# abdur75648/AI-Camera

Measured on AMD Instinct MI355X. Metric: end-to-end frames/sec @1280x720, 30 persons/frame, higher is better.
Workload: dtype f16

## Files before the change

### ai-camera_amd/csrc/conv_common.hpp

```cpp
#pragma once
#include "kernels.hpp"

#include <cstdlib>
#include <type_traits>
#include <utility>

namespace aic {

typedef _Float16 half8 __attribute__((ext_vector_type(8)));
typedef _Float16 half4 __attribute__((ext_vector_type(4)));
typedef float floatx4 __attribute__((ext_vector_type(4)));

__device__ __forceinline__ float act_apply(float v, int act) {
    if (act == 1) return v / (1.0f + __expf(-v));
    if (act == 2) return fmaxf(v, 0.0f);
    return v;
}

template <typename T> struct Frag;
template <> struct Frag<half_t> {
    typedef half8 type;
    static __device__ __forceinline__ floatx4 mma(const half8& a, const half8& b, floatx4 c) {
        return __builtin_amdgcn_mfma_f32_16x16x32_f16(a, b, c, 0, 0, 0);
    }
};
template <> struct Frag<float> {
    typedef floatx4 type;
    static __device__ __forceinline__ floatx4 partial(const floatx4& a, const floatx4& b) {
        floatx4 p = {0.f, 0.f, 0.f, 0.f};
        p = __builtin_amdgcn_mfma_f32_16x16x4f32(a[0], b[0], p, 0, 0, 0);
        p = __builtin_amdgcn_mfma_f32_16x16x4f32(a[1], b[1], p, 0, 0, 0);
        p = __builtin_amdgcn_mfma_f32_16x16x4f32(a[2], b[2], p, 0, 0, 0);
        p = __builtin_amdgcn_mfma_f32_16x16x4f32(a[3], b[3], p, 0, 0, 0);
        return p;
    }
    static __device__ __forceinline__ floatx4 mma(const floatx4& a, const floatx4& b, floatx4 c) { return c + partial(a, b); }
};

template <typename T, int MT, int NT>
__device__ __forceinline__ void mma_tiles(floatx4 (&acc)[MT][NT], const typename Frag<T>::type (&wf)[NT], const typename Frag<T>::type (&xf)[MT]) {
    if constexpr (sizeof(T) == 2) {
#pragma unroll
        for (int i = 0; i < MT; ++i)
#pragma unroll
            for (int j = 0; j < NT; ++j) acc[i][j] = Frag<T>::mma(wf[j], xf[i], acc[i][j]);
    } else {
        floatx4 prev = Frag<T>::partial(wf[0], xf[0]);
        __builtin_amdgcn_sched_barrier(0);
#pragma unroll
        for (int t = 1; t < MT * NT; ++t) {
            const floatx4 p = Frag<T>::partial(wf[t % NT], xf[t / NT]);
            acc[(t - 1) / NT][(t - 1) % NT] += prev;
            asm volatile("" : "+v"(acc[(t - 1) / NT][(t - 1) % NT]));
            prev = p;
            __builtin_amdgcn_sched_barrier(0);
        }
        acc[MT - 1][NT - 1] += prev;
        asm volatile("" : "+v"(acc[MT - 1][NT - 1]));
    }
}

constexpr int MID_STEPS = 16;
template <int MT, int NT>
__device__ __forceinline__ void mma_tiles_mid(floatx4 (&mid)[MT][NT], const floatx4 (&wf)[NT], const floatx4 (&xf)[MT]) {
    floatx4 prev = Frag<float>::partial(wf[0], xf[0]);
    __builtin_amdgcn_sched_barrier(0);
#pragma unroll
    for (int t = 1; t < MT * NT; ++t) {
        const floatx4 p = Frag<float>::partial(wf[t % NT], xf[t / NT]);
        mid[(t - 1) / NT][(t - 1) % NT] += prev;
        asm volatile("" : "+v"(mid[(t - 1) / NT][(t - 1) % NT]));
        prev = p;
        __builtin_amdgcn_sched_barrier(0);
    }
    mid[MT - 1][NT - 1] += prev;
    asm volatile("" : "+v"(mid[MT - 1][NT - 1]));
}
typedef float doublex4 __attribute__((ext_vector_type(4)));
template <int MT, int NT>
__device__ __forceinline__ void flush_mid(doublex4 (&accd)[MT][NT], floatx4 (&mid)[MT][NT]) {
#pragma unroll
    for (int i = 0; i < MT; ++i)
#pragma unroll
        for (int j = 0; j < NT; ++j) {
#pragma unroll
            for (int e = 0; e < 4; ++e) accd[i][j][e] += mid[i][j][e];
            mid[i][j] = floatx4{0.f, 0.f, 0.f, 0.f};
        }
}

__device__ __forceinline__ int lds_swz(int row) { return ((row >> 1) & 3) ^ ((row >> 3) & 2); }
__device__ __forceinline__ int lds_off(int row, int chunk) { return row * 64 + 16 * (chunk ^ lds_swz(row)); }

__device__ __forceinline__ void fast_divmod(int m, int d, float inv, int& q, int& r) {
    q = (int)(__int2float_rz(m) * inv);
    r = m - q * d;
    if (r >= d) { r -= d; ++q; }
    if (r < 0) { r += d; --q; }
}

template <int ACT> __device__ __forceinline__ float act_fast(float v) {
    if constexpr (ACT == 1) {
        return v * __builtin_amdgcn_rcpf(1.0f + __builtin_amdgcn_exp2f(v * -1.4426950408889634f));
    } else if constexpr (ACT == 2) {
        return fmaxf(v, 0.0f);
    } else {
        return v;
    }
}

template <typename T, int ACT> __device__ __forceinline__ float act_t(float v) {
    if constexpr (sizeof(T) == 4 && ACT == 1) return v / (1.0f + expf(-v));
    else return act_fast<ACT>(v);
}

template <typename T, int MT, int NT, int ACT, int RES, bool F32OUT>
__device__ __forceinline__ void epilogue_fast(const ConvArgs& a, floatx4 (&acc)[MT][NT], const int (&mrow)[MT], int n_base, int q) {
    const float* __restrict__ bias = a.bias;
    const T* __restrict__ rg = reinterpret_cast<const T*>(a.res);
    floatx4 b4[NT];
    bool ncol[NT];
#pragma unroll
    for (int j = 0; j < NT; ++j) {
        const int n = n_base + j * 16 + 4 * q;
        ncol[j] = n < a.Cout;
        b4[j] = *reinterpret_cast<const floatx4*>(bias + n);
    }
#pragma unroll
    for (int i = 0; i < MT; ++i) {
        const int m = mrow[i];
        if (m < 0) continue;
        const size_t ybase = (size_t)m * a.y_cs + a.y_coff;
        const size_t rbase = RES ? (size_t)m * a.r_cs + a.r_coff : 0;
#pragma unroll
        for (int j = 0; j < NT; ++j) {
            if (!ncol[j]) continue;
            const int n = n_base + j * 16 + 4 * q;
            float v[4];
#pragma unroll
            for (int e = 0; e < 4; ++e) v[e] = acc[i][j][e] + b4[j][e];
            if constexpr (RES != 0) {
                float rv[4];
                if constexpr (sizeof(T) == 2) {
                    const half4 h = *reinterpret_cast<const half4*>(rg + rbase + n);
#pragma unroll
                    for (int e = 0; e < 4; ++e) rv[e] = (float)h[e];
                } else {
                    const floatx4 h = *reinterpret_cast<const floatx4*>(rg + rbase + n);
#pragma unroll
                    for (int e = 0; e < 4; ++e) rv[e] = h[e];
                }
#pragma unroll
                for (int e = 0; e < 4; ++e) v[e] = RES == 1 ? act_t<T, ACT>(v[e] + rv[e]) : act_t<T, ACT>(v[e]) + rv[e];
            } else {
// ... 292 lines not shown
#pragma unroll
            for (int e = 0; e < 4; ++e) own[e] = (half_t)act_fast<1>(acc[i][NT - 1][e] + b1[NT - 1][e]);
            const int2 u = *reinterpret_cast<const int2*>(&own);
            const int s0 = (((2 * q) & 3) * 16 + r) * 4, s1 = (((2 * q + 1) & 3) * 16 + r) * 4;
            int4 g;
            g.x = __builtin_amdgcn_ds_bpermute(s0, u.x), g.y = __builtin_amdgcn_ds_bpermute(s0, u.y);
            g.z = __builtin_amdgcn_ds_bpermute(s1, u.x), g.w = __builtin_amdgcn_ds_bpermute(s1, u.y);
            if (q >= 2) g = make_int4(0, 0, 0, 0);
            bf[NP] = *reinterpret_cast<const half8*>(&g);
        }
        floatx4 acc2[1][NT];
#pragma unroll
        for (int j = 0; j < NT; ++j) acc2[0][j] = floatx4{0.f, 0.f, 0.f, 0.f};
#pragma unroll
        for (int s = 0; s < KS; ++s)
#pragma unroll
            for (int j = 0; j < NT; ++j) acc2[0][j] = __builtin_amdgcn_mfma_f32_16x16x32_f16(wf[j][s], bf[s], acc2[0][j], 0, 0, 0);
        const int m1[1] = {mrow[i]};
        if (a.t_max) {
            floatx4 bt[NT];
#pragma unroll
            for (int p = 0; p < NP; ++p) {
                bt[2 * p] = *reinterpret_cast<const floatx4*>(a.b_tail + 32 * p + 8 * q);
                bt[2 * p + 1] = *reinterpret_cast<const floatx4*>(a.b_tail + 32 * p + 8 * q + 4);
            }
            if constexpr (NT & 1) bt[NT - 1] = *reinterpret_cast<const floatx4*>(a.b_tail + 16 * (NT - 1) + 4 * q);
            float best = -__builtin_inff();
            int arg = 0x7fffffff;
#pragma unroll
            for (int j = 0; j < NT; ++j)
#pragma unroll
                for (int e = 0; e < 4; ++e) {
                    const int ch = perm_ch<NT>(j, q, e);
                    const float v = acc2[0][j][e] + bt[j][e];
                    if (ch < a.t_cout && v > best) { best = v; arg = ch; }
                }
#pragma unroll
            for (int off = 16; off <= 32; off <<= 1) {
                const float ov = __shfl_xor(best, off);
                const int oa = __shfl_xor(arg, off);
                if (ov > best || (ov == best && oa < arg)) { best = ov; arg = oa; }
            }
            const int m = mrow[i];
            if (q == 0 && m >= 0) {
                const int im = m / a.t_hw;
                const size_t o = (size_t)im * a.t_na + a.t_a0 + (m - im * a.t_hw);
                a.t_max[o] = best;
                a.t_arg[o] = arg;
            }
        } else if (NT == 4 && a.t_box) {
            if constexpr (NT == 4) {
                floatx4 bt[4];
#pragma unroll
                for (int p = 0; p < 2; ++p) {
                    bt[2 * p] = *reinterpret_cast<const floatx4*>(a.b_tail + 32 * p + 8 * q);
                    bt[2 * p + 1] = *reinterpret_cast<const floatx4*>(a.b_tail + 32 * p + 8 * q + 4);
                }
                const bool odd = q & 1;
                float dist[2];
#pragma unroll
                for (int h = 0; h < 2; ++h) {
                    float v[8];
#pragma unroll
                    for (int k = 0; k < 8; ++k) v[k] = acc2[0][2 * h + (k >> 2)][k & 3] + bt[2 * h + (k >> 2)][k & 3];
                    float mx = v[0];
#pragma unroll
                    for (int k = 1; k < 8; ++k) mx = fmaxf(mx, v[k]);
                    mx = fmaxf(mx, __shfl_xor(mx, 16));
                    float e[8];
#pragma unroll
                    for (int k = 0; k < 8; ++k) e[k] = __builtin_amdgcn_exp2f((v[k] - mx) * 1.4426950408889634f);
                    float sum = 0.f, ex = 0.f;
                    if (!odd) {
#pragma unroll
                        for (int k = 0; k < 8; ++k) { sum += e[k]; ex += e[k] * (float)k; }
                    }
                    const float s_in = __shfl_xor(sum, 16), x_in = __shfl_xor(ex, 16);
                    if (odd) {
                        sum = s_in, ex = x_in;
#pragma unroll
                        for (int k = 0; k < 8; ++k) { sum += e[k]; ex += e[k] * (float)(8 + k); }
                    }
                    dist[h] = ex / sum;
                }
                const float d1 = __shfl_xor(dist[0], 32), d3 = __shfl_xor(dist[1], 32);
                const int m = mrow[i];
                if (q == 1 && m >= 0) {
                    const int im = m / a.t_hw, cell = m - im * a.t_hw;
                    const int gy = cell / a.t_w, gx = cell - gy * a.t_w;
                    const float cx = (float)gx + 0.5f, cy = (float)gy + 0.5f, st = (float)a.t_stride;
                    const size_t o = (size_t)im * a.t_na + a.t_a0 + cell;
                    *reinterpret_cast<floatx4*>(a.t_box + o * 4) = floatx4{(cx - dist[0]) * st, (cy - d1) * st, (cx + dist[1]) * st, (cy + d3) * st};
                }
            }
        } else {
            epilogue_dispatch<half_t, 1, NT, true>(a2, acc2, m1, 0, q);
        }
    }
}

typedef const __attribute__((address_space(1))) void* gptr_t;
typedef __attribute__((address_space(3))) void* lptr_t;


__device__ __forceinline__ int xcd_tile(int b, int nb, int on) {
    if (!on) return b;
    const int x = b & 7, base = nb >> 3, rem = nb & 7;
    return x * base + (x < rem ? x : rem) + (b >> 3);
}
__device__ __forceinline__ void xcd_tile_xy(int on, int& bx, int& by) {
    const int nbx = (int)gridDim.x, lin = (int)blockIdx.y * nbx + (int)blockIdx.x;
    const int t = xcd_tile(lin, nbx * (int)gridDim.y, on);
    by = t / nbx, bx = t - by * nbx;
}
__device__ __forceinline__ bool xcd_tile_xy_live(int on, int nbx_live, int& bx, int& by) {
    const int lin = (int)blockIdx.y * (int)gridDim.x + (int)blockIdx.x;
    const int nlive = nbx_live * (int)gridDim.y;
    if (lin >= nlive) return false;
    const int t = xcd_tile(lin, nlive, on);
    by = t / nbx_live, bx = t - by * nbx_live;
    return true;
}

template <int N> __device__ __forceinline__ void wait_vmcnt() {
    if constexpr (N == 0) asm volatile("s_waitcnt vmcnt(0)" ::: "memory");
    else if constexpr (N == 1) asm volatile("s_waitcnt vmcnt(1)" ::: "memory");
    else if constexpr (N == 2) asm volatile("s_waitcnt vmcnt(2)" ::: "memory");
    else if constexpr (N == 3) asm volatile("s_waitcnt vmcnt(3)" ::: "memory");
    else if constexpr (N == 4) asm volatile("s_waitcnt vmcnt(4)" ::: "memory");
    else if constexpr (N == 5) asm volatile("s_waitcnt vmcnt(5)" ::: "memory");
    else if constexpr (N == 6) asm volatile("s_waitcnt vmcnt(6)" ::: "memory");
    else if constexpr (N == 7) asm volatile("s_waitcnt vmcnt(7)" ::: "memory");
    else if constexpr (N == 8) asm volatile("s_waitcnt vmcnt(8)" ::: "memory");
    else if constexpr (N == 9) asm volatile("s_waitcnt vmcnt(9)" ::: "memory");
    else if constexpr (N == 10) asm volatile("s_waitcnt vmcnt(10)" ::: "memory");
    else if constexpr (N == 11) asm volatile("s_waitcnt vmcnt(11)" ::: "memory");
    else if constexpr (N == 12) asm volatile("s_waitcnt vmcnt(12)" ::: "memory");
    else if constexpr (N == 14) asm volatile("s_waitcnt vmcnt(14)" ::: "memory");
    else if constexpr (N == 15) asm volatile("s_waitcnt vmcnt(15)" ::: "memory");
    else if constexpr (N == 16) asm volatile("s_waitcnt vmcnt(16)" ::: "memory");
    else if constexpr (N == 18) asm volatile("s_waitcnt vmcnt(18)" ::: "memory");
    else if constexpr (N == 20) asm volatile("s_waitcnt vmcnt(20)" ::: "memory");
    else static_assert(N < 0, "add this vmcnt literal");
}


constexpr int ppp_ipix_pad(int th, int tw) {
    int ipix = (th + 2) * (tw + 2);
    if (tw >= 16) return ipix;
    while (ipix % 16 != tw && ipix % 16 != 16 - tw) ++ipix;
    return ipix;
}

__device__ __forceinline__ int lane_here() {
    int l;
    asm volatile("v_mbcnt_lo_u32_b32 %0, -1, 0\n\tv_mbcnt_hi_u32_b32 %0, -1, %0" : "=v"(l));
    return l;
}


void launch_conv_wide(const ConvArgs& a, const ConvPlan& p, hipStream_t s);
void launch_conv_pp(const ConvArgs& a, const ConvPlan& p, hipStream_t s);
void launch_conv_pp_patch(const ConvArgs& a, const ConvPlan& p, hipStream_t s);
void launch_conv_sp_patch(const ConvArgs& a, const ConvPlan& p, hipStream_t s);
void launch_conv_s2_patch(const ConvArgs& a, const ConvPlan& p, hipStream_t s);
void launch_conv_patch(const ConvArgs& a, const ConvPlan& p, hipStream_t s);
void launch_conv_pm_patch(const ConvArgs& a, const ConvPlan& p, hipStream_t s);
void launch_conv_c16(const ConvArgs& a, const ConvPlan& p, hipStream_t s);
void launch_conv_c32s2_tail(const ConvArgs& a, const ConvPlan& p, hipStream_t s);
void launch_conv_1x1_stream(const ConvArgs& a, const ConvPlan& p, hipStream_t s);
void launch_conv_c64_resident(const ConvArgs& a, const ConvPlan& p, hipStream_t s);

}
```

### ai-camera_amd/csrc/kernels_conv_sp.hip

```cpp
#include "conv_common.hpp"

namespace aic {

template <int MT, int NT, int WM, int WN, int TH, int TW>
__global__ __launch_bounds__(512) void conv3x3_sp_patch_kernel(const ConvArgs a, int ny, int run) {
    typedef half_t T;
    constexpr int NSTAGE = 4;
    constexpr int CH = 8, BKE = 32, RP = 128;
    constexpr int BM = WM * MT * 16;
    constexpr int BN = WN * NT * 16;
    constexpr int B_PER = BN / RP;
    constexpr int LPS = B_PER + 1;
    constexpr int TPIX = TH * TW, NI = BM / TPIX;
    constexpr int PW = TW + 2, PH = TH + 2, IPIX = PW * PH, IPIXP = ppp_ipix_pad(TH, TW), NPIX = NI * IPIXP;
    constexpr int G = TW >= 16 ? 1 : 16 / TW;
    constexpr int NPASS = (NPIX + 127) / 128, NPIXP = NPASS * 128;
    constexpr int PLANE = NPIXP * 16, PBUF = 4 * PLANE, WSTAGE = BN * 64;
    constexpr int PATCH0 = NSTAGE * WSTAGE, DUM0 = PATCH0 + 2 * PBUF;
    static_assert(WM * WN == 8 && MT == 8 && NT == 4 && BN % RP == 0 && BM % TPIX == 0 && NPASS <= 7 && TW % 4 == 0, "geometry");
    static_assert((NSTAGE - 1) * WSTAGE + 2048 < 65536 && PBUF + (2 * PW + 2 + IPIXP * NI) * 16 < 65536, "ds_read immediates");

    extern __shared__ __attribute__((aligned(16))) char smem[];

    const int t = threadIdx.x;
    const int lane = t & 63, wv = __builtin_amdgcn_readfirstlane(t >> 6);
    const int HW = a.H * a.W;
    const int n_img = a.n_dev ? min(a.M / HW, a.n_dev[0]) : a.M / HW;
    const int ntiles = ((n_img + NI - 1) / NI) * ny;
    const int nruns = (ntiles + run - 1) / run;
    if ((int)blockIdx.x >= nruns) return;
    int t_cur = xcd_tile((int)blockIdx.x, nruns, a.xcd_map) * run;
    const int t_end = min(t_cur + run, ntiles);
    int img0 = (t_cur / ny) * NI, n0 = (t_cur % ny) * BN;

    const T* __restrict__ xg = reinterpret_cast<const T*>(a.x);
    const T* __restrict__ wg = reinterpret_cast<const T*>(a.w);
    const T* zero = reinterpret_cast<const T*>(a.zero);

    const int plane = wv & 3;
    const T* pptr[NPASS];
    int pil[NPASS];
#pragma unroll
    for (int i = 0; i < NPASS; ++i) {
        const int p = i * 128 + (wv >> 2) * 64 + lane;
        const int il = p / IPIXP, rem = p - il * IPIXP;
        const int py = rem / PW, px = rem - py * PW;
        const int iy = py - 1, ix = px - 1;
        const bool ok = p < NPIX && rem < IPIX && (unsigned)iy < (unsigned)TH && (unsigned)ix < (unsigned)TW;
        pptr[i] = ok ? xg + ((size_t)((il * TH + iy) * TW + ix) * a.x_cs + a.x_coff + plane * CH) : zero;
        pil[i] = ok ? il : 0x40000000;
    }
    char* const pdst = smem + PATCH0 + plane * PLANE + (wv >> 2) * 1024;
    const unsigned img_bytes = (unsigned)HW * a.x_cs * 2u;
    const int slot = t & 3, r0 = t >> 2;
    const int kc = slot ^ lds_swz(r0);
    const T* wptr[B_PER];
#pragma unroll
    for (int j = 0; j < B_PER; ++j) wptr[j] = wg + (size_t)(r0 + RP * j) * a.Kp + kc * CH;
    char* const wdst = smem + (16 * wv) * 64;
    const int nchunks = a.Cin / BKE;
    const unsigned tile_wbytes = (unsigned)BN * a.Kp * 2u;
    const unsigned tap_bytes = (unsigned)a.Cin * 2u;

    unsigned long long w_off = (unsigned long long)(n0 / BN) * tile_wbytes;
    int w_c = 0;
    int n0_next = n0, img_next = img0;
    bool has_next = t_cur + 1 < t_end;
    if (has_next) { img_next = ((t_cur + 1) / ny) * NI; n0_next = ((t_cur + 1) % ny) * BN; }
    auto issue_w = [&](int st, int wtap) {
        char* sbase = wdst + st * WSTAGE;
#pragma unroll
        for (int j = 0; j < B_PER; ++j) {
            const T* src = reinterpret_cast<const T*>(reinterpret_cast<const char*>(wptr[j]) + w_off);
            asm volatile("" : "+v"(src));
            __builtin_amdgcn_global_load_lds((gptr_t)src, (lptr_t)(sbase + j * (RP * 64)), 16, 0, 0);
        }
        if (wtap < 8) w_off += tap_bytes;
        else {
            w_off += 64u - 8u * (unsigned long long)tap_bytes;
            if (++w_c == nchunks) {
                w_c = 0;
                w_off = (unsigned long long)((has_next ? n0_next : n0) / BN) * tile_wbytes;
            }
        }
    };
    unsigned long long p_off = 0;
    int p_lim = 0;
    auto set_patch = [&](int c) {
        const bool inner = c + 1 < nchunks;
        const int im = inner ? img0 : img_next;
        p_off = (unsigned long long)im * img_bytes + (inner ? (unsigned)(c + 1) * 64u : 0u);
        p_lim = (inner || has_next) ? n_img - im : 0;
    };
    auto issue_patch = [&](auto ic, int buf) {
        constexpr int i = decltype(ic)::value;
        const bool live = pil[i] < p_lim;
        const unsigned lo = live ? (unsigned)p_off : 0u, hi = live ? (unsigned)(p_off >> 32) : 0u;
        const T* src = reinterpret_cast<const T*>(reinterpret_cast<const char*>(pptr[i]) + (((unsigned long long)hi << 32) | lo));
        asm volatile("" : "+v"(src));
        __builtin_amdgcn_global_load_lds((gptr_t)src, (lptr_t)(pdst + buf * PBUF + i * 2048), 16, 0, 0);
    };
    auto issue_dummy = [&] {
        const T* src = zero;
        asm volatile("" : "+v"(src));
        __builtin_amdgcn_global_load_lds((gptr_t)src, (lptr_t)(smem + DUM0 + wv * 1024), 16, 0, 0);
    };

    const int wm = wv / WN, wn = wv % WN;
    const int q = lane >> 4, r = lane & 15;
    static_assert((MT * 16) % TPIX == 0 || TPIX % (MT * 16) == 0, "a wave's pixels must not straddle images irregularly");
    static_assert(TW % 16 == 0 || 16 % TW == 0, "a 16-pixel MFMA tile is whole rows or a piece of one row");
    static_assert(G == 1 || (NI % G == 0 && (MT % TH == 0 || TH % MT == 0)), "image groups");
    auto tile_pix = [](int t) constexpr { return G == 1 ? (t * 16 / TPIX) * IPIXP + ((t * 16 % TPIX) / TW) * PW + (t * 16 % TPIX) % TW
                                                        : (t / TH) * G * IPIXP + (t % TH) * PW; };
    auto patch_pix = [tile_pix](int m) constexpr { return G == 1 ? tile_pix(m / 16) : (TH % MT == 0 ? (m / 16) * PW : tile_pix(m / 16)); };
    int xa0;
    if constexpr (G == 1) {
        const int ml = wm * MT * 16 + r;
        const int il = ml / TPIX, rem = ml - il * TPIX;
        const int ly = rem / TW, lx = rem - ly * TW;
        xa0 = PATCH0 + q * PLANE + (il * IPIXP + ly * PW + lx) * 16;
    } else {
        const int t0 = wm * MT;
        xa0 = PATCH0 + q * PLANE + ((t0 / TH) * G * IPIXP + (t0 % TH) * PW + (r / TW) * IPIXP + r % TW) * 16;
    }
    int woff2[2];
#pragma unroll
    for (int j = 0; j < 2; ++j) woff2[j] = lds_off(wn * NT * 16 + perm_row<NT>(j, r), q);

    floatx4 acc[MT][NT];
    half8 xf[MT], wf[2][NT];
    auto read_w = [&](auto setc, int st) {
        constexpr int S = decltype(setc)::value;
#pragma unroll
        for (int j = 0; j < NT; ++j) wf[S][j] = *reinterpret_cast<const half8*>(smem + woff2[j & 1] + st * WSTAGE + (j >> 1) * 2048);
    };
    auto read_x = [&](int i, int buf, int tap) {
        xf[i] = *reinterpret_cast<const half8*>(smem + xa0 + buf * PBUF + ((tap / 3) * PW + tap % 3) * 16 + patch_pix(16 * i) * 16);
    };

    p_off = (unsigned long long)img0 * img_bytes, p_lim = n_img - img0;
    static_for<NPASS>([&](auto ic) { issue_patch(ic, 0); });
#pragma unroll
    for (int st = 0; st < NSTAGE - 1; ++st) {
        issue_w(st, st);
        if (st) issue_dummy();
    }
    wait_vmcnt<LPS>();
    __builtin_amdgcn_s_barrier();

    auto body = [&](int c, auto c4c, auto tapc) {
        constexpr int C4 = decltype(c4c)::value, tap = decltype(tapc)::value;
        constexpr int BUF = C4 & 1, ST = (C4 + tap) & 3, CUR = ST & 1, NXT = CUR ^ 1;
        constexpr int nbuf = tap < 8 ? BUF : BUF ^ 1, ntap = tap < 8 ? tap + 1 : 0;
        if constexpr (tap == 0) set_patch(c);
        static_for<MT>([&](auto ic) {
            constexpr int i = decltype(ic)::value;
#pragma unroll
            for (int j = 0; j < NT; ++j)
                asm volatile("v_mfma_f32_16x16x32_f16 %0, %1, %2, %0" : "+v"(acc[i][j]) : "v"(wf[CUR][j]), "v"(xf[i]));
            read_x(i, nbuf, ntap);
            if constexpr (i == 0) read_w(std::integral_constant<int, NXT>{}, (ST + 1) & 3);
            if constexpr (i == 1) issue_w((ST + 3) & 3, (tap + 3) % 9);
            if constexpr (i == 2) {
                if constexpr (tap < NPASS) issue_patch(tapc, BUF ^ 1);
                else issue_dummy();
            }
            __builtin_amdgcn_sched_barrier(0);
        });
        __builtin_amdgcn_s_waitcnt(0x0070 | LPS);
        __builtin_amdgcn_s_barrier();
    };
    for (;;) {
#pragma unroll
        for (int i = 0; i < MT; ++i)
#pragma unroll
            for (int j = 0; j < NT; ++j) acc[i][j] = floatx4{0.f, 0.f, 0.f, 0.f};
        read_w(std::integral_constant<int, 0>{}, 0);
#pragma unroll
        for (int i = 0; i < MT; ++i) read_x(i, 0, 0);
        __builtin_amdgcn_s_waitcnt(0xC07F);
        for (int c = 0; c < nchunks; c += 4) {
            static_for<4>([&](auto c4c) {
                static_for<9>([&](auto tapc) { body(c + decltype(c4c)::value, c4c, tapc); });
            });
        }
        if (!has_next) wait_vmcnt<0>();
        asm volatile("s_nop 15\n\ts_nop 15" ::: "memory");

        int mrow[MT];
        const int ln = lane_here(), rr = ln & 15, qe = ln >> 4;
#pragma unroll
        for (int i = 0; i < MT; ++i) {
            int il, ly, lx;
            if constexpr (G == 1) {
                const int ml = (wm * MT + i) * 16 + rr;
                il = ml / TPIX;
                const int rem = ml - il * TPIX;
                ly = rem / TW, lx = rem - ly * TW;
            } else {
                const int tl = wm * MT + i;
                il = (tl / TH) * G + rr / TW, ly = tl % TH, lx = rr % TW;
            }
            const int img = img0 + il;
            mrow[i] = img < n_img ? (img * TH + ly) * TW + lx : -1;
        }
        epilogue_dispatch<T, MT, NT, true, true>(a, acc, mrow, n0 + wn * NT * 16, qe);
        if (!has_next) break;
        ++t_cur;
        img0 = img_next, n0 = n0_next;
        has_next = t_cur + 1 < t_end;
        if (has_next) { img_next = ((t_cur + 1) / ny) * NI; n0_next = ((t_cur + 1) % ny) * BN; }
    }
}

template <int MT, int NT, int WM, int WN, int TH, int TW>
static void launch_sp_patch(const ConvArgs& a, const ConvPlan& p, hipStream_t s) {
    constexpr int BM = WM * MT * 16, BN = WN * NT * 16;
    constexpr int NI = BM / (TH * TW), NPIX = NI * ppp_ipix_pad(TH, TW), NPASS = (NPIX + 127) / 128;
    constexpr size_t lds = (size_t)2 * 4 * NPASS * 128 * 16 + 8192 + (size_t)4 * BN * 64;
    static_assert(lds <= 160 * 1024, "does not fit the LDS");
    auto kfn = conv3x3_sp_patch_kernel<MT, NT, WM, WN, TH, TW>;
    set_lds_limit(kfn, lds);
    hipLaunchKernelGGL(kfn, dim3((unsigned)p.blocks), dim3(512), lds, s, a, a.Cout / BN, p.run);
    KCHECK();
}


template <int NPASS> struct S2dSched;
template <> struct S2dSched<5> { static constexpr int n[9][4] = {{1,1,0,0},{1,1,0,0},{0,2,0,0},{0,0,2,0},{0,0,3,0},{0,0,0,3},{0,0,0,2},{2,0,0,0},{1,1,0,0}}; };
template <> struct S2dSched<3> { static constexpr int n[9][4] = {{1,0,0,0},{0,1,0,0},{0,1,0,0},{0,1,1,0},{0,0,2,0},{0,0,0,2},{0,0,0,1},{1,0,0,0},{1,0,0,0}}; };

template <int WM, int WN, int TH, int TW>
__global__ __launch_bounds__(512) void conv3x3s2_sp_patch_kernel(const ConvArgs a, int ny, int run) {
    typedef half_t T;
    constexpr int MT = 8, NT = 4, NSTAGE = 4;
    constexpr int CH = 8, BKE = 32, RP = 128;
    constexpr int BM = WM * MT * 16, BN = WN * NT * 16, B_PER = BN / RP;
    constexpr int TPIX = TH * TW, NI = BM / TPIX;
    constexpr int PW = TW + 2, PH = TH + 2, IPIX = PW * PH, IPIXP = ppp_ipix_pad(TH, TW), NPIX = NI * IPIXP;
    constexpr int G = TW >= 16 ? 1 : 16 / TW;
    constexpr int NPASS = (NPIX + 127) / 128, NPIXP = NPASS * 128;
    constexpr int PLANE = NPIXP * 16, PBUF = 4 * PLANE, WSTAGE = BN * 64;
    constexpr int PATCH0 = NSTAGE * WSTAGE;
    typedef S2dSched<NPASS> SCH;
    static_assert(WM * WN == 8 && BN % RP == 0 && BM % TPIX == 0 && TW % 4 == 0, "geometry");
    static_assert((PW + 1 + IPIXP * NI) * 16 < 65536, "ds_read immediates");
    constexpr int H = 2 * TH, W = 2 * TW;

    extern __shared__ __attribute__((aligned(16))) char smem[];
    const int t = threadIdx.x;
    const int lane = t & 63, wv = __builtin_amdgcn_readfirstlane(t >> 6);
    const int n_img = a.n_dev ? min(a.M / TPIX, a.n_dev[0]) : a.M / TPIX;
    const int ntiles = ((n_img + NI - 1) / NI) * ny;
    const int nruns = (ntiles + run - 1) / run;
    if ((int)blockIdx.x >= nruns) return;
    int t_cur = xcd_tile((int)blockIdx.x, nruns, a.xcd_map) * run;
    const int t_end = min(t_cur + run, ntiles);
    int img0 = (t_cur / ny) * NI, n0 = (t_cur % ny) * BN;

    const T* __restrict__ xg = reinterpret_cast<const T*>(a.x);
    const T* __restrict__ wg = reinterpret_cast<const T*>(a.w);
    const T* zero = reinterpret_cast<const T*>(a.zero);

    const int plane = wv & 3;
    unsigned poff[NPASS];
#pragma unroll
    for (int i = 0; i < NPASS; ++i) {
        const int p = i * 128 + (wv >> 2) * 64 + lane;
        const int il = p / IPIXP, rem = p - il * IPIXP;
        const int py = rem / PW, px = rem - py * PW;
        const int va = py - 1, vb = px - 1;
        const bool ok = p < NPIX && rem < IPIX && (unsigned)va < (unsigned)TH && (unsigned)vb < (unsigned)TW;
        poff[i] = ok ? (unsigned)((((il * H + 2 * va) * W + 2 * vb) * a.x_cs + a.x_coff + plane * CH) * 2) : 0xffffffffu;
    }
    char* const pdst = smem + PATCH0 + plane * PLANE + (wv >> 2) * 1024;
    const unsigned img_bytes = (unsigned)(H * W) * a.x_cs * 2u;
    const int slot = t & 3, r0 = t >> 2;
    const int kc = slot ^ lds_swz(r0);
    const T* wptr[B_PER];
#pragma unroll
    for (int j = 0; j < B_PER; ++j) wptr[j] = wg + (size_t)(r0 + RP * j) * a.Kp + kc * CH;
    char* const wdst = smem + (16 * wv) * 64;
    const int nh = a.Cin / BKE;
    const unsigned tile_wbytes = (unsigned)BN * a.Kp * 2u, tap_bytes = (unsigned)a.Cin * 2u;

    int n0_next = n0, img_next = img0;
    bool has_next = t_cur + 1 < t_end;
    if (has_next) { img_next = ((t_cur + 1) / ny) * NI; n0_next = ((t_cur + 1) % ny) * BN; }

    constexpr int PL_[9] = {0, 0, 0, 0, 1, 1, 2, 2, 3};
    constexpr int KH_[9] = {0, 0, 1, 1, 0, 1, 1, 1, 1}, KW_[9] = {0, 1, 0, 1, 1, 1, 0, 1, 1};
    constexpr int TAP_[9] = {0, 2, 6, 8, 1, 7, 3, 5, 4};
    constexpr int CPI_[4] = {1, 1, 0, 0}, CPJ_[4] = {1, 0, 1, 0};

    auto issue_w = [&](int st, int nn, int hh, int tapi) {
        unsigned long long w_off = (unsigned long long)(nn / BN) * tile_wbytes + (unsigned long long)tapi * tap_bytes + (unsigned)hh * 64u;
        asm volatile("" : "+s"(w_off));
#pragma unroll
        for (int j = 0; j < B_PER; ++j) {
            const T* src = reinterpret_cast<const T*>(reinterpret_cast<const char*>(wptr[j]) + w_off);
            asm volatile("" : "+v"(src));
            __builtin_amdgcn_global_load_lds((gptr_t)src, (lptr_t)(wdst + st * WSTAGE + j * (RP * 64)), 16, 0, 0);
        }
    };
    auto udiv24 = [](int x, auto dc) { constexpr int D = decltype(dc)::value; constexpr unsigned Mg = (1u << 24) / D + 1u; return (int)(__umul24((unsigned)x, Mg) >> 24); };
    auto issue_patch = [&](auto ic, int buf, int im, int lim, int pi, int pj, int hh) {
        constexpr int i = decltype(ic)::value;
        unsigned long long base = (unsigned long long)reinterpret_cast<uintptr_t>(xg) + (unsigned long long)im * img_bytes +
                                  (unsigned long long)(((pi * W + pj) * a.x_cs + hh * BKE) * 2);
        asm volatile("" : "+s"(base));
        int il = 0;
        if constexpr (NI > 1) il = udiv24(i * 128 + (wv >> 2) * 64 + lane_here(), std::integral_constant<int, IPIXP>{});
        const bool live = poff[i] != 0xffffffffu && il < lim;
        const unsigned long long addr = base + poff[i];
        const unsigned long long zaddr = (unsigned long long)reinterpret_cast<uintptr_t>(zero);
        const T* src = reinterpret_cast<const T*>(live ? addr : zaddr);
        asm volatile("" : "+v"(src));
        __builtin_amdgcn_global_load_lds((gptr_t)src, (lptr_t)(pdst + buf * PBUF + i * 2048), 16, 0, 0);
    };

    const int wm = wv / WN, wn = wv % WN;
    const int q = lane >> 4, r = lane & 15;
    static_assert((MT * 16) % TPIX == 0 || TPIX % (MT * 16) == 0, "a wave's pixels must not straddle images irregularly");
    static_assert(TW % 16 == 0 || 16 % TW == 0, "a 16-pixel MFMA tile is whole rows or a piece of one row");
    static_assert(G == 1 || (NI % G == 0 && (MT % TH == 0 || TH % MT == 0)), "image groups");
    auto tile_pix = [](int t) constexpr { return G == 1 ? (t * 16 / TPIX) * IPIXP + ((t * 16 % TPIX) / TW) * PW + (t * 16 % TPIX) % TW
                                                        : (t / TH) * G * IPIXP + (t % TH) * PW; };
    auto patch_pix = [tile_pix](int m) constexpr { return G == 1 ? tile_pix(m / 16) : (TH % MT == 0 ? (m / 16) * PW : tile_pix(m / 16)); };
    int xa0;
    if constexpr (G == 1) {
        const int ml = wm * MT * 16 + r;
        const int il = ml / TPIX, rem = ml - il * TPIX;
        const int ly = rem / TW, lx = rem - ly * TW;
        xa0 = PATCH0 + q * PLANE + (il * IPIXP + ly * PW + lx) * 16;
    } else {
        const int t0 = wm * MT;
        xa0 = PATCH0 + q * PLANE + ((t0 / TH) * G * IPIXP + (t0 % TH) * PW + (r / TW) * IPIXP + r % TW) * 16;
    }
    int woff2[2];
#pragma unroll
    for (int j = 0; j < 2; ++j) woff2[j] = lds_off(wn * NT * 16 + perm_row<NT>(j, r), q);

    floatx4 acc[MT][NT];
    half8 xf[MT], wf[2][NT];
    auto read_w = [&](auto setc, int st) {
        constexpr int S = decltype(setc)::value;
        const int w0 = woff2[0] + st * WSTAGE, w1 = woff2[1] + st * WSTAGE;
#pragma unroll
        for (int j = 0; j < NT; ++j) wf[S][j] = *reinterpret_cast<const half8*>(smem + ((j & 1) ? w1 : w0) + (j >> 1) * 2048);
    };
    auto read_x = [&](int i, int xaddr, int kh, int kw) {
        xf[i] = *reinterpret_cast<const half8*>(smem + xaddr + (kh * PW + kw) * 16 + patch_pix(16 * i) * 16);
    };

    int st = 0;
    int bufc = 0;
    {
        const int lim = n_img - img0;
        static_for<NPASS>([&](auto ic) { issue_patch(ic, 0, img0, lim, 1, 1, 0); });
        static_for<NPASS>([&](auto ic) {
            constexpr int i = decltype(ic)::value;
            if constexpr (i < SCH::n[7][0] + SCH::n[8][0]) issue_patch(ic, 1, img0, lim, 1, 0, 0);
            if constexpr (i < SCH::n[8][1]) issue_patch(ic, 2, img0, lim, 0, 1, 0);
        });
        issue_w(0, n0, 0, TAP_[0]);
        issue_w(1, n0, 0, TAP_[1]);
        wait_vmcnt<0>();
        issue_w(2, n0, 0, TAP_[2]);
        __builtin_amdgcn_s_barrier();
    }

    auto body = [&](int h, auto parc, auto bc) {
        constexpr int PAR = decltype(parc)::value, b = decltype(bc)::value;
        constexpr int CUR = (PAR + b) & 1, NXT = CUR ^ 1;
        constexpr int nb = (b + 1) % 9;
        constexpr bool new_chunk = PL_[nb] != PL_[b];
        const int buf_next = new_chunk ? (bufc == 2 ? 0 : bufc + 1) : bufc;
        const int xaddr = xa0 + buf_next * PBUF;
        const int st_n = (st + 1) & 3, st_w = (st + 3) & 3;
        constexpr int wb = (b + 3) % 9;
        int w_h = h + (b + 3 >= 9 ? 1 : 0), w_n = n0;
        if (w_h == nh) { w_h = 0; w_n = has_next ? n0_next : n0; }
        constexpr int n1 = SCH::n[b][0], n2 = SCH::n[b][1], n3 = SCH::n[b][2], n4 = SCH::n[b][3];
        constexpr int LPS_B = B_PER + n1 + n2 + n3 + n4;
        auto before = [](int tgt, int bb) constexpr {
            constexpr int start[4] = {7, 8, 3, 5};
            int cnt = 0;
            for (int k = start[tgt]; k != bb; k = (k + 1) % 9) cnt += SCH::n[k][tgt];
            return cnt;
        };
        constexpr bool nextp1 = b >= 7, nextp2 = b >= 8;
        int t_h[4] = {h + (nextp1 ? 1 : 0), h + (nextp2 ? 1 : 0), h, h + 1}, t_im[4], t_lim[4];
#pragma unroll
        for (int k = 0; k < 4; ++k) {
            const bool over = t_h[k] >= nh;
            t_im[k] = over ? img_next : img0;
            t_lim[k] = over ? (has_next ? n_img - img_next : 0) : n_img - img0;
            t_h[k] = over ? 0 : t_h[k];
        }
        constexpr int ct = PL_[b];
        constexpr int ahead[4] = {((nextp1 ? 4 : 0) + 1 - ct + 3) % 3, ((nextp2 ? 4 : 0) + 2 - ct + 3) % 3, (3 - ct) % 3, (4 - ct) % 3};
        auto tbuf = [&](int k) { const int v = bufc + ahead[k]; return v >= 3 ? v - 3 : v; };
        static_for<MT>([&](auto ic) {
            constexpr int i = decltype(ic)::value;
#pragma unroll
            for (int j = 0; j < NT; ++j)
                asm volatile("v_mfma_f32_16x16x32_f16 %0, %1, %2, %0" : "+v"(acc[i][j]) : "v"(wf[CUR][j]), "v"(xf[i]));
            read_x(i, xaddr, KH_[nb], KW_[nb]);
            if constexpr (i == 0) read_w(std::integral_constant<int, NXT>{}, st_n);
            if constexpr (i == 1) issue_w(st_w, w_n, w_h, TAP_[wb]);
            if constexpr (i == 2) {
                static_for<NPASS>([&](auto pc) {
                    constexpr int pi_ = decltype(pc)::value;
                    if constexpr (pi_ >= before(0, b) && pi_ < before(0, b) + n1) issue_patch(pc, tbuf(0), t_im[0], t_lim[0], CPI_[1], CPJ_[1], t_h[0]);
                    if constexpr (pi_ >= before(1, b) && pi_ < before(1, b) + n2) issue_patch(pc, tbuf(1), t_im[1], t_lim[1], CPI_[2], CPJ_[2], t_h[1]);
                    if constexpr (pi_ >= before(2, b) && pi_ < before(2, b) + n3) issue_patch(pc, tbuf(2), t_im[2], t_lim[2], CPI_[3], CPJ_[3], t_h[2]);
                    if constexpr (pi_ >= before(3, b) && pi_ < before(3, b) + n4) issue_patch(pc, tbuf(3), t_im[3], t_lim[3], CPI_[0], CPJ_[0], t_h[3]);
                });
            }
            __builtin_amdgcn_sched_barrier(0);
        });
        st = st_n;
        bufc = buf_next;
        __builtin_amdgcn_s_waitcnt(0x0070 | LPS_B);
        __builtin_amdgcn_s_barrier();
    };
    for (;;) {
#pragma unroll
        for (int i = 0; i < MT; ++i)
#pragma unroll
            for (int j = 0; j < NT; ++j) acc[i][j] = floatx4{0.f, 0.f, 0.f, 0.f};
        read_w(std::integral_constant<int, 0>{}, st);
        {
            const int xaddr = xa0 + bufc * PBUF;
#pragma unroll
            for (int i = 0; i < MT; ++i) read_x(i, xaddr, 0, 0);
        }
        __builtin_amdgcn_s_waitcnt(0xC07F);
        for (int h = 0; h < nh; h += 2) {
            static_for<9>([&](auto bc) { body(h, std::integral_constant<int, 0>{}, bc); });
            static_for<9>([&](auto bc) { body(h + 1, std::integral_constant<int, 1>{}, bc); });
        }
        if (!has_next) wait_vmcnt<0>();
        asm volatile("s_nop 15\n\ts_nop 15" ::: "memory");

        int mrow[MT];
        const int ln = lane_here(), rr = ln & 15, qe = ln >> 4;
#pragma unroll
        for (int i = 0; i < MT; ++i) {
            int il, ly, lx;
            if constexpr (G == 1) {
                const int ml = (wm * MT + i) * 16 + rr;
                il = ml / TPIX;
                const int rem = ml - il * TPIX;
                ly = rem / TW, lx = rem - ly * TW;
            } else {
                const int tl = wm * MT + i;
                il = (tl / TH) * G + rr / TW, ly = tl % TH, lx = rr % TW;
            }
            const int img = img0 + il;
            mrow[i] = img < n_img ? (img * TH + ly) * TW + lx : -1;
        }
        epilogue_dispatch<T, MT, NT, true, true>(a, acc, mrow, n0 + wn * NT * 16, qe);
        if (!has_next) break;
        ++t_cur;
        img0 = img_next, n0 = n0_next;
        has_next = t_cur + 1 < t_end;
        if (has_next) { img_next = ((t_cur + 1) / ny) * NI; n0_next = ((t_cur + 1) % ny) * BN; }
    }
}

template <int WM, int WN, int TH, int TW>
static void launch_s2_patch(const ConvArgs& a, const ConvPlan& p, hipStream_t s) {
    constexpr int BM = WM * 128, BN = WN * 64;
    constexpr int NI = BM / (TH * TW), NPIX = NI * ppp_ipix_pad(TH, TW), NPASS = (NPIX + 127) / 128;
    constexpr size_t lds = (size_t)3 * 4 * NPASS * 128 * 16 + (size_t)4 * BN * 64;
    static_assert(lds <= 160 * 1024, "does not fit the LDS");
    auto kfn = conv3x3s2_sp_patch_kernel<WM, WN, TH, TW>;
    set_lds_limit(kfn, lds);
    hipLaunchKernelGGL(kfn, dim3((unsigned)p.blocks), dim3(512), lds, s, a, a.Cout / BN, p.run);
    KCHECK();
}

void launch_conv_s2_patch(const ConvArgs& a, const ConvPlan& p, hipStream_t s) {
    if (p.wm == 4 && p.wn == 2 && p.th == 32 && p.tw == 16) return launch_s2_patch<4, 2, 32, 16>(a, p, s);
    if (p.wm == 2 && p.wn == 4 && p.th == 16 && p.tw == 8) return launch_s2_patch<2, 4, 16, 8>(a, p, s);
    AIC_REQUIRE(false, AIC_ERR_INVALID, "conv plan: no stride-2 patch instantiation for this tile");
}

void launch_conv_sp_patch(const ConvArgs& a, const ConvPlan& p, hipStream_t s) {
    const bool t84 = p.mt == 8 && p.nt == 4;
    if (t84 && p.wm == 4 && p.wn == 2 && p.th == 32 && p.tw == 16) return launch_sp_patch<8, 4, 4, 2, 32, 16>(a, p, s);
    if (t84 && p.wm == 2 && p.wn == 4 && p.th == 16 && p.tw == 8) return launch_sp_patch<8, 4, 2, 4, 16, 8>(a, p, s);
    if (t84 && p.wm == 2 && p.wn == 4 && p.th == 8 && p.tw == 4) return launch_sp_patch<8, 4, 2, 4, 8, 4>(a, p, s);
    AIC_REQUIRE(false, AIC_ERR_INVALID, "conv plan: no software-pipelined patch instantiation for this tile");
}

}
```

Measured before the change: 12730.

## Remap sp-patch MFMA tiles to image columns and skip padding-only taps

```diff
diff --git a/ai-camera_amd/csrc/conv_common.hpp b/ai-camera_amd/csrc/conv_common.hpp
--- a/ai-camera_amd/csrc/conv_common.hpp
+++ b/ai-camera_amd/csrc/conv_common.hpp
@@ -1,5 +1,6 @@
 #pragma once
 #include "kernels.hpp"
+#include "pad_skip_map.hpp"
 
 #include <cstdlib>
 #include <type_traits>
@@ -598,6 +599,12 @@
     return ipix;
 }
 
+template <int TH, int TW, int NI, int WM, int MT, bool COL> struct PatchGeom {
+    static constexpr int PW = TW + 2, IPIXP = ppp_ipix_pad(TH, TW);
+    static constexpr bool skip(int, int) { return false; }
+};
+template <int TH, int TW, int NI, int WM, int MT> struct PatchGeom<TH, TW, NI, WM, MT, true> : ColTiles<TH, TW, NI, WM, MT> {};
+
 __device__ __forceinline__ int lane_here() {
     int l;
     asm volatile("v_mbcnt_lo_u32_b32 %0, -1, 0\n\tv_mbcnt_hi_u32_b32 %0, -1, %0" : "=v"(l));
diff --git a/ai-camera_amd/csrc/kernels_conv_sp.hip b/ai-camera_amd/csrc/kernels_conv_sp.hip
--- a/ai-camera_amd/csrc/kernels_conv_sp.hip
+++ b/ai-camera_amd/csrc/kernels_conv_sp.hip
@@ -2,7 +2,7 @@
 
 namespace aic {
 
-template <int MT, int NT, int WM, int WN, int TH, int TW>
+template <int MT, int NT, int WM, int WN, int TH, int TW, bool COL = false>
 __global__ __launch_bounds__(512) void conv3x3_sp_patch_kernel(const ConvArgs a, int ny, int run) {
     typedef half_t T;
     constexpr int NSTAGE = 4;
@@ -12,7 +12,8 @@
     constexpr int B_PER = BN / RP;
     constexpr int LPS = B_PER + 1;
     constexpr int TPIX = TH * TW, NI = BM / TPIX;
-    constexpr int PW = TW + 2, PH = TH + 2, IPIX = PW * PH, IPIXP = ppp_ipix_pad(TH, TW), NPIX = NI * IPIXP;
+    typedef PatchGeom<TH, TW, NI, WM, MT, COL> GEO;
+    constexpr int PW = GEO::PW, PH = TH + 2, IPIX = PW * PH, IPIXP = GEO::IPIXP, NPIX = NI * IPIXP;
     constexpr int G = TW >= 16 ? 1 : 16 / TW;
     constexpr int NPASS = (NPIX + 127) / 128, NPIXP = NPASS * 128;
     constexpr int PLANE = NPIXP * 16, PBUF = 4 * PLANE, WSTAGE = BN * 64;
@@ -115,7 +116,9 @@
                                                         : (t / TH) * G * IPIXP + (t % TH) * PW; };
     auto patch_pix = [tile_pix](int m) constexpr { return G == 1 ? tile_pix(m / 16) : (TH % MT == 0 ? (m / 16) * PW : tile_pix(m / 16)); };
     int xa0;
-    if constexpr (G == 1) {
+    if constexpr (COL) {
+        xa0 = PATCH0 + q * PLANE + (GEO::wave_off(wm) + GEO::lane_off(r)) * 16;
+    } else if constexpr (G == 1) {
         const int ml = wm * MT * 16 + r;
         const int il = ml / TPIX, rem = ml - il * TPIX;
         const int ly = rem / TW, lx = rem - ly * TW;
@@ -136,7 +139,10 @@
         for (int j = 0; j < NT; ++j) wf[S][j] = *reinterpret_cast<const half8*>(smem + woff2[j & 1] + st * WSTAGE + (j >> 1) * 2048);
     };
     auto read_x = [&](int i, int buf, int tap) {
-        xf[i] = *reinterpret_cast<const half8*>(smem + xa0 + buf * PBUF + ((tap / 3) * PW + tap % 3) * 16 + patch_pix(16 * i) * 16);
+        int toff;
+        if constexpr (COL) toff = GEO::tile_off(i);
+        else toff = patch_pix(16 * i);
+        xf[i] = *reinterpret_cast<const half8*>(smem + xa0 + buf * PBUF + ((tap / 3) * PW + tap % 3) * 16 + toff * 16);
     };
 
     p_off = (unsigned long long)img0 * img_bytes, p_lim = n_img - img0;
@@ -156,10 +162,12 @@
         if constexpr (tap == 0) set_patch(c);
         static_for<MT>([&](auto ic) {
             constexpr int i = decltype(ic)::value;
-#pragma unroll
-            for (int j = 0; j < NT; ++j)
-                asm volatile("v_mfma_f32_16x16x32_f16 %0, %1, %2, %0" : "+v"(acc[i][j]) : "v"(wf[CUR][j]), "v"(xf[i]));
-            read_x(i, nbuf, ntap);
+            if constexpr (!GEO::skip(i, tap)) {
+#pragma unroll
+                for (int j = 0; j < NT; ++j)
+                    asm volatile("v_mfma_f32_16x16x32_f16 %0, %1, %2, %0" : "+v"(acc[i][j]) : "v"(wf[CUR][j]), "v"(xf[i]));
+            }
+            if constexpr (!GEO::skip(i, ntap)) read_x(i, nbuf, ntap);
             if constexpr (i == 0) read_w(std::integral_constant<int, NXT>{}, (ST + 1) & 3);
             if constexpr (i == 1) issue_w((ST + 3) & 3, (tap + 3) % 9);
             if constexpr (i == 2) {
@@ -193,7 +201,9 @@
 #pragma unroll
         for (int i = 0; i < MT; ++i) {
             int il, ly, lx;
-            if constexpr (G == 1) {
+            if constexpr (COL) {
+                il = GEO::img(wm, i, rr), ly = GEO::y(rr), lx = GEO::x(i);
+            } else if constexpr (G == 1) {
                 const int ml = (wm * MT + i) * 16 + rr;
                 il = ml / TPIX;
                 const int rem = ml - il * TPIX;
@@ -214,13 +224,13 @@
     }
 }
 
-template <int MT, int NT, int WM, int WN, int TH, int TW>
+template <int MT, int NT, int WM, int WN, int TH, int TW, bool COL = false>
 static void launch_sp_patch(const ConvArgs& a, const ConvPlan& p, hipStream_t s) {
     constexpr int BM = WM * MT * 16, BN = WN * NT * 16;
-    constexpr int NI = BM / (TH * TW), NPIX = NI * ppp_ipix_pad(TH, TW), NPASS = (NPIX + 127) / 128;
+    constexpr int NI = BM / (TH * TW), NPIX = NI * PatchGeom<TH, TW, NI, WM, MT, COL>::IPIXP, NPASS = (NPIX + 127) / 128;
     constexpr size_t lds = (size_t)2 * 4 * NPASS * 128 * 16 + 8192 + (size_t)4 * BN * 64;
     static_assert(lds <= 160 * 1024, "does not fit the LDS");
-    auto kfn = conv3x3_sp_patch_kernel<MT, NT, WM, WN, TH, TW>;
+    auto kfn = conv3x3_sp_patch_kernel<MT, NT, WM, WN, TH, TW, COL>;
     set_lds_limit(kfn, lds);
     hipLaunchKernelGGL(kfn, dim3((unsigned)p.blocks), dim3(512), lds, s, a, a.Cout / BN, p.run);
     KCHECK();
@@ -491,9 +501,12 @@
 
 void launch_conv_sp_patch(const ConvArgs& a, const ConvPlan& p, hipStream_t s) {
     const bool t84 = p.mt == 8 && p.nt == 4;
+    static const bool col = getenv("AICAM_NO_PAD_SKIP") == nullptr;
     if (t84 && p.wm == 4 && p.wn == 2 && p.th == 32 && p.tw == 16) return launch_sp_patch<8, 4, 4, 2, 32, 16>(a, p, s);
-    if (t84 && p.wm == 2 && p.wn == 4 && p.th == 16 && p.tw == 8) return launch_sp_patch<8, 4, 2, 4, 16, 8>(a, p, s);
-    if (t84 && p.wm == 2 && p.wn == 4 && p.th == 8 && p.tw == 4) return launch_sp_patch<8, 4, 2, 4, 8, 4>(a, p, s);
+    if (t84 && p.wm == 2 && p.wn == 4 && p.th == 16 && p.tw == 8)
+        return col ? launch_sp_patch<8, 4, 2, 4, 16, 8, true>(a, p, s) : launch_sp_patch<8, 4, 2, 4, 16, 8>(a, p, s);
+    if (t84 && p.wm == 2 && p.wn == 4 && p.th == 8 && p.tw == 4)
+        return col ? launch_sp_patch<8, 4, 2, 4, 8, 4, true>(a, p, s) : launch_sp_patch<8, 4, 2, 4, 8, 4>(a, p, s);
     AIC_REQUIRE(false, AIC_ERR_INVALID, "conv plan: no software-pipelined patch instantiation for this tile");
 }
 
diff --git a/ai-camera_amd/csrc/pad_skip_map.hpp b/ai-camera_amd/csrc/pad_skip_map.hpp
--- /dev/null
+++ b/ai-camera_amd/csrc/pad_skip_map.hpp
@@ -0,0 +1,28 @@
+#pragma once
+
+namespace aic {
+
+template <int TH, int TW, int NI, int WM = 2, int MT = 8>
+struct ColTiles {
+    static constexpr int CG = 16 / TH;
+    static constexpr int IW = NI / WM;
+    static constexpr int PW = TW + 3, PH = TH + 2;
+    static constexpr int IPIX = PW * PH;
+    static constexpr int IPIXP = CG == 1 ? IPIX : IPIX + (8 - IPIX % 16 + 16) % 16;
+    static constexpr int NPIX = NI * IPIXP, NPASS = (NPIX + 127) / 128;
+    static_assert(16 % TH == 0 && TH >= 8 && TW % 2 == 0 && NI % WM == 0 && IW % CG == 0, "a tile is one column of one or two whole images");
+    static_assert(MT * CG == TW * IW, "a wave's MT tiles are the TW columns of its IW / CG image groups");
+    static_assert(PW % 2 == 1 && (CG == 1 || IPIXP % 16 == 8), "bank slots");
+
+    static constexpr int wave_off(int wm) { return wm * IW * IPIXP; }
+    static constexpr int tile_off(int i) { return (i / TW) * CG * IPIXP + i % TW; }
+    static constexpr int lane_off(int r) { return (r / TH) * IPIXP + (r % TH) * PW; }
+    static constexpr int tap_off(int tap) { return (tap / 3) * PW + tap % 3; }
+    static constexpr int img(int wm, int i, int r) { return wm * IW + (i / TW) * CG + r / TH; }
+    static constexpr int y(int r) { return r % TH; }
+    static constexpr int x(int i) { return i % TW; }
+    static constexpr bool skip(int i, int tap) { return (tap % 3 == 0 && x(i) == 0) || (tap % 3 == 2 && x(i) == TW - 1); }
+    static constexpr int max_off() { return wave_off(WM - 1) + tile_off(MT - 1) + lane_off(15) + tap_off(8); }
+};
+
+}
```

Result: faster. 12870, median of 6 (+1.1%).
